# SRainGit/CAE-LO

Hardware: AMD Instinct MI355X
Metric: KITTI frames/sec end-to-end (keypts+desc+match+RANSAC) (higher is better)
Workload: dtype f32

## Files before the change

### cae-lo_amd/csrc/caelo_internal.h

```cpp
#pragma once
#include <hip/hip_runtime.h>
#include <stdint.h>
#include <stdio.h>
#include <string.h>

#include "../../include/caelo.h"

#define CAELO_API extern "C" __attribute__((visibility("default")))

void caelo_set_error(const char *fmt, ...);

#define CAELO_HIP(expr)                                                                     \
    do {                                                                                    \
        hipError_t _e = (expr);                                                             \
        if (_e != hipSuccess) {                                                             \
            caelo_set_error("%s:%d: %s failed: %s", __FILE__, __LINE__, #expr, hipGetErrorString(_e)); \
            return CAELO_ERR_HIP;                                                           \
        }                                                                                   \
    } while (0)

#define CAELO_LAUNCH_CHECK()                                                                \
    do {                                                                                    \
        hipError_t _e = hipGetLastError();                                                  \
        if (_e != hipSuccess) {                                                             \
// ... 188 lines not shown
}
#endif
int certify_record(const caelo_ransac_cert &c, const double *rnd, caelo_pose_result *res, uint8_t *mask, int64_t mask_len, int32_t *evals);

struct caelo_clear_item {
    void *ptr;
    size_t bytes;
    uint32_t pattern;
};
#define CAELO_CLEAR_MAX 12
struct caelo_clear_list {
    caelo_clear_item item[CAELO_CLEAR_MAX];
    int n;
};
int caelo_clear_many(const caelo_clear_list &list, hipStream_t s);
int caelo_clear_many_set(const caelo_clear_list *lists, int n_frames, hipStream_t s);

int ring_project_launch(const float *pc, int64_t n, float *ring, int32_t *counter, int32_t *winner, int32_t *status,
                        hipStream_t s);
int ring_respond_launch(caelo_ctx *c, const float *in, int in_w, int in_c, float *resp, hipStream_t s);
int ring_keypoints_launch(const float *ring, int ring_w, int ring_c, int dist_c, const int32_t *counter, int cnt_w,
                          const float *resp, unsigned long long *cand, int32_t *cand_count,
                          int64_t *key_pixels, float *key_pts, int kp_ld, float *valid, int valid_ld, int32_t *n_key,
                          int32_t *status, hipStream_t s);
int ring_project_set(const caelo_frame_set &fs, hipStream_t s);
int ring_respond_set(caelo_ctx *c, const caelo_frame_set &fs, int in_w, int in_c, hipStream_t s, int row0, int rows);
int ring_keypoints_set(const caelo_frame_set &fs, int ring_w, int ring_c, int cnt_w, hipStream_t s);
void vox_clear_items(caelo_voxmap *m, int level, caelo_clear_list &list);
int vox_clear_for_fast_build(caelo_voxmap *m, caelo_clear_list &list, hipStream_t s);
int vox_clear_for_fast_build_set(caelo_voxmap *const *maps, int n, caelo_clear_list *lists, hipStream_t s);
int vox_build_fast_set(caelo_voxmap *const *maps, const caelo_frame_set &fs, hipStream_t s);
int vox_build_set(caelo_voxmap *const *maps, const caelo_frame_set &fs, bool track_order, hipStream_t s);
int vox_patches_set(const caelo_frame_set &fs, int64_t k_max, bool check_counts, hipStream_t s);
int dedup_set(const caelo_frame_set &fs, bool enabled, hipStream_t s);
int vox_build_launch(caelo_voxmap *m, const float *pc, int64_t n, int stride, bool track_order, int32_t *status,
                     hipStream_t s);
int vox_build_fast_launch(caelo_voxmap *m, const float *pc, int64_t n, int stride, int32_t *status, hipStream_t s);
int vox_patches_launch(const caelo_voxmap *m, const float *pts, int pts_ld, int64_t k_max, const int32_t *n_key,
                       uint64_t *bits, uint8_t *flags, int32_t *status, bool check_counts, hipStream_t s,
                       void *dedup_scratch = nullptr);
#define CAELO_FRAME_PATCHES (CAELO_MAX_KEYPTS * 3)
struct caelo_dedup_tables {
    int32_t count;
    int32_t pad[63];
    int32_t list[CAELO_FRAME_PATCHES];
    int32_t slot_of[CAELO_FRAME_PATCHES];
};
#define CAELO_FRAME_BITS_BYTES ((size_t)CAELO_FRAME_PATCHES * 64 * 8)
#define CAELO_FRAME_BUF_BYTES (CAELO_FRAME_BITS_BYTES + sizeof(caelo_dedup_tables))
__host__ __device__ inline caelo_dedup_tables *caelo_frame_tables(const uint64_t *frame_bits) {
    return (caelo_dedup_tables *)((char *)frame_bits + CAELO_FRAME_BITS_BYTES);
}
#define DD_SLOTS_FRAME 8192
#define DD_SLOTS_SET 65536
#define DD_EMPTY 0xFFFFFFFFFFFFFFFFull
struct DedupScratch {
    unsigned long long table[DD_SLOTS_SET];
    int32_t pslot[CAELO_FRAME_PATCHES];
    int32_t rep[CAELO_FRAME_PATCHES];
};
__host__ __device__ inline uint32_t dedup_slot_mask(int n_frames) { return (n_frames > 1 ? DD_SLOTS_SET : DD_SLOTS_FRAME) - 1; }
int64_t dedup_scratch_bytes();
void dedup_clear_item(void *scratch, int n_frames, caelo_clear_list &list);
unsigned long long dedup_hash_mask();
bool dedup_enabled(int mode);
int dedup_launch(uint64_t *frame_bits, void *scratch, bool enabled, hipStream_t s);

#define CAELO_ENC_MAX_FRAMES CAELO_FB_MAX
struct caelo_enc_out {
    float *base[CAELO_ENC_MAX_FRAMES];
    int64_t per_frame;
};
#define CAELO_ENC_WS_HEADER 4096
#define CAELO_ENC_WS_MFMA 3072
struct caelo_enc_in {
    const unsigned long long *bits;
    int64_t frame_stride;
    int32_t per_frame, n_frames, dedup;
    int32_t yield;
};
__device__ inline const caelo_dedup_tables *enc_tables(const caelo_enc_in &in, int f) {
    return (const caelo_dedup_tables *)(in.bits + (size_t)f * in.frame_stride + (size_t)in.per_frame * 64);
}
int encode_batch_impl(caelo_ctx *c, const uint64_t *bits, int64_t n_patches, int group, const caelo_enc_out &outs,
                      int out_stride, void *ws, hipStream_t s, hipEvent_t *ev, const caelo_enc_in *in = nullptr);
int64_t enc_dense_pad(int64_t n);
int enc_upload_dense1(const float *wd1, const float *bd1, int K, void **wx_dev, float **bd_dev);
int64_t enc_dense32_part_bytes(int64_t np);
int enc_dense32_head_launch(caelo_ctx *c, const float *f3, int64_t n_patches, int64_t np, float *part, int group, float *out,
                            int out_stride, hipStream_t s);
int encode_impl(caelo_ctx *c, const uint64_t *bits, int64_t n_patches, int group, float *out, int out_stride, void *ws,
                hipStream_t s, hipEvent_t *ev);

struct caelo_extract_args {
    caelo_ctx *ctx;
    caelo_voxmap *map;
    const float *pc;
    int64_t n;
    int dist_channels, mode;
    float *key_pts;
    int kp_ld;
    float *features;
    int feat_ld;
    float *valid;
    int valid_ld;
    int64_t *key_pixels;
    int32_t *n_key;
    uint8_t *flags;
    int32_t *status;
    void *ws;
    uint64_t *bits;
};
int extract_check(const caelo_extract_args &a);
int extract_front_launch(const caelo_extract_args &a, hipStream_t s);
int extract_front_set(const caelo_extract_args *args, int n, hipStream_t s, hipStream_t s_vox = nullptr, hipEvent_t ev_fork = nullptr,
                      hipEvent_t ev_join = nullptr);
int extract_encode_launch(const caelo_extract_args &a, hipStream_t s);
int exact_patches_prepare(caelo_voxmap *const *maps, int n_frames);
void exact_patches_clear_item(caelo_voxmap *m, caelo_clear_list &list);
int exact_patches_redo(caelo_voxmap *const *maps, const caelo_frame_set &fs, const caelo_extract_args *args, int n, hipStream_t s);

int correct_prepare(caelo_voxmap *const *maps, int n);
int correct_set(const caelo_extract_args *args, int n, hipStream_t s);

#define CAELO_KP_HIST_BINS 2048

__device__ inline void caelo_frame_block(int n_frames, unsigned &frame, unsigned &block, unsigned &per_frame) {
    per_frame = gridDim.x / (unsigned)n_frames;
    if ((n_frames & (n_frames - 1)) == 0) {
        frame = blockIdx.x & (unsigned)(n_frames - 1);
        block = blockIdx.x / (unsigned)n_frames;
    } else {
        frame = blockIdx.x / per_frame;
        block = blockIdx.x - frame * per_frame;
    }
}

__device__ inline void caelo_lds_barrier() { __asm__ volatile("s_waitcnt lgkmcnt(0)\n\ts_barrier" ::: "memory"); }

__host__ __device__ inline unsigned long long caelo_pack3(int x, int y, int z) {
    return ((unsigned long long)(unsigned)(x & 0xFFFFF) << 40) | ((unsigned long long)(unsigned)(y & 0xFFFFF) << 20) |
           (unsigned long long)(unsigned)(z & 0xFFFFF);
}

__device__ inline uint32_t caelo_hash64(unsigned long long k) {
    k ^= k >> 33;
    k *= 0xff51afd7ed558ccdULL;
    k ^= k >> 33;
    k *= 0xc4ceb9fe1a85ec53ULL;
    k ^= k >> 33;
    return (uint32_t)k;
}

__device__ inline unsigned long long caelo_dd_mix(unsigned long long k) {
    k ^= k >> 33;
    k *= 0xff51afd7ed558ccdULL;
    k ^= k >> 33;
    k *= 0xc4ceb9fe1a85ec53ULL;
    k ^= k >> 33;
    return k;
}
__device__ inline void caelo_dedup_insert(unsigned long long word, int lane, int p, int gp, DedupScratch *S, DedupScratch *T, uint32_t slot_mask,
                                          unsigned long long hash_mask) {
    unsigned long long h = caelo_dd_mix(word + 0x9E3779B97F4A7C15ull * (unsigned)(lane + 1));
#pragma unroll
    for (int o = 32; o > 0; o >>= 1) h += __shfl_xor(h, o);
    if (lane != 0) return;
    h = caelo_dd_mix(h) & hash_mask & 0xFFFFFFFFFEull;
// ... 65 lines not shown
```

### cae-lo_amd/csrc/encoder.hip

```cpp
#include <math.h>

#include "caelo_internal.h"
#include <vector>
#include <stdlib.h>
#include <string.h>

typedef float f32x4 __attribute__((ext_vector_type(4)));

#define MFMA16(a, b, c) __builtin_amdgcn_mfma_f32_16x16x4f32((a), (b), (c), 0, 0, 0)

__device__ inline float enc_tanh(float x) {
    const float e = __builtin_amdgcn_exp2f(x * 2.8853900817779268f);
    return 1.0f - 2.0f * __builtin_amdgcn_rcpf(e + 1.0f);
}

#define DENSE_N 200
#define DENSE_NP 208
#define DENSE_K 2048
#define C3X_NPAIR 14
#define C3X_TICKET_INT 512
static void conv3_split_weights(const float *w3, uint4 *out);
static void stage1x_split_weights(const float *w1, const float *w2, uint4 *w1f, uint4 *w2x);
int enc_upload_dense1(const float *wd1, const float *bd1, int K, void **wx_dev, float **bd_dev);
#define HEAD_WQ_FLOATS (13 * 2 * 64 * 4)
// ... 940 lines not shown
    const float *src = part + (size_t)row * DENSE_NP + 4 * g;
    float4 v[HM_JW][SPLIT];
#pragma unroll
    for (int c = 0; c < HM_JW; ++c)
#pragma unroll
        for (int sp = 0; sp < SPLIT; ++sp)
            if (wave + 4 * c < D1_NT) v[c][sp] = *(const float4 *)(src + (size_t)sp * n_rows_pad * DENSE_NP + 16 * (wave + 4 * c));
    f32x4 acc0 = {0.f, 0.f, 0.f, 0.f}, acc1 = {0.f, 0.f, 0.f, 0.f};
#pragma unroll
    for (int c = 0; c < HM_JW; ++c) {
        if (wave + 4 * c < D1_NT) {
            float4 sum = b1[c];
#pragma unroll
            for (int sp = 0; sp < SPLIT; ++sp) { sum.x += v[c][sp].x; sum.y += v[c][sp].y; sum.z += v[c][sp].z; sum.w += v[c][sp].w; }
            const float hv[4] = {enc_tanh(sum.x), enc_tanh(sum.y), enc_tanh(sum.z), enc_tanh(sum.w)};
            const float w0[4] = {wq[c][0].x, wq[c][0].y, wq[c][0].z, wq[c][0].w}, w1[4] = {wq[c][1].x, wq[c][1].y, wq[c][1].z, wq[c][1].w};
#pragma unroll
            for (int i = 0; i < 4; ++i) {
                acc0 = __builtin_amdgcn_mfma_f32_16x16x4f32(hv[i], w0[i], acc0, 0, 0, 0);
                acc1 = __builtin_amdgcn_mfma_f32_16x16x4f32(hv[i], w1[i], acc1, 0, 0, 0);
            }
        }
    }
    if (wave > 0) {
        s_c[wave - 1][0][lane] = acc0;
        s_c[wave - 1][1][lane] = acc1;
    }
    __syncthreads();
    if (wave > 0) return;
#pragma unroll
    for (int w = 0; w < 3; ++w) {
        acc0 += s_c[w][0][lane];
        acc1 += s_c[w][1][lane];
    }
    const float bo0 = bd2[m], bo1 = m < 4 ? bd2[16 + m] : 0.0f;
#pragma unroll
    for (int i = 0; i < 4; ++i) {
        const unsigned pp = tile * 16u + 4u * (unsigned)g + (unsigned)i;
        if (pp < n_all) {
            const unsigned f = pp / per_out, q = pp - f * per_out, kp = q / (unsigned)group;
            float *dst = outs.base[f] + (size_t)kp * out_stride + (size_t)(q - kp * (unsigned)group) * 20;
            const float d0 = enc_tanh(bo0 + acc0[i]);
            dst[m] = d0;
            if (!(fabsf(d0) <= 1.0f)) atomicAdd(faults, 1);
            if (m < 4) {
                const float d1 = enc_tanh(bo1 + acc1[i]);
                dst[16 + m] = d1;
                if (!(fabsf(d1) <= 1.0f)) atomicAdd(faults, 1);
            }
        }
    }
}

static inline int64_t pad64(int64_t n) { return (n + D1_BM - 1) / D1_BM * D1_BM; }


CAELO_API int64_t caelo_encode_ws_bytes(int64_t n_patches) {
    const int64_t np = pad64(n_patches);
    return CAELO_ENC_WS_HEADER + (np * 1024 + np * 2048 + (int64_t)D1_SPLIT * np * DENSE_NP) * (int64_t)sizeof(float);
}

CAELO_API int caelo_encode_ws_layout(int64_t n_patches, int64_t out[6]) {
    CAELO_REQUIRE(out && n_patches > 0, "caelo_encode_ws_layout: bad argument");
    const int64_t np = pad64(n_patches);
    out[0] = CAELO_ENC_WS_HEADER;
    out[1] = out[0] + np * 1024 * (int64_t)sizeof(float);
    out[2] = out[1] + np * 2048 * (int64_t)sizeof(float);
    out[3] = np;
    out[4] = D1_SPLIT_OF(DENSE_K);
    out[5] = D1_SPLIT;
    return CAELO_OK;
}

int encode_impl(caelo_ctx *c, const uint64_t *bits, int64_t n_patches, int group, float *out, int out_stride,
                       void *ws, hipStream_t s, hipEvent_t *ev ) {
    CAELO_REQUIRE(out, "null argument");
    caelo_enc_out outs;
    outs.base[0] = out;
    outs.per_frame = n_patches > 0 ? n_patches : 1;
    return encode_batch_impl(c, bits, n_patches, group, outs, out_stride, ws, s, ev);
}

int encode_batch_impl(caelo_ctx *c, const uint64_t *bits, int64_t n_patches, int group, const caelo_enc_out &outs,
                      int out_stride, void *ws, hipStream_t s, hipEvent_t *ev , const caelo_enc_in *in) {
    CAELO_REQUIRE(c && bits && ws, "null argument");
    const caelo_enc_in ein = in ? *in : caelo_enc_in{(const unsigned long long *)bits, 0, (int32_t)(n_patches < 0x7FFFFFFF ? n_patches : 0), 1, 0, 0};
    CAELO_REQUIRE(!ein.dedup || (ein.n_frames >= 1 && ein.n_frames <= CAELO_ENC_MAX_FRAMES && ein.per_frame % (3 * D1_BM) == 0 &&
                                 (int64_t)ein.n_frames * ein.per_frame == n_patches),
                  "bad de-duplicated launch");
    CAELO_REQUIRE(outs.per_frame > 0 && (n_patches + outs.per_frame - 1) / outs.per_frame <= CAELO_ENC_MAX_FRAMES, "bad frame table");
    CAELO_REQUIRE(!ein.dedup || ein.per_frame == CAELO_FRAME_PATCHES, "de-duplicated launches hold whole frames of 3072 patches");
    CAELO_REQUIRE(c->has_enc, "encoder weights not set (caelo_set_encoder_weights)");
    CAELO_REQUIRE(n_patches > 0 && n_patches < 0x7FFFFFFF && group >= 1 && out_stride >= group * 20, "bad shape");
    const int64_t np = pad64(n_patches);
    int *work_counter = (int *)ws;
    unsigned long long *mfma_count = (unsigned long long *)((char *)ws + CAELO_ENC_WS_MFMA);
    float *p2 = (float *)((char *)ws + CAELO_ENC_WS_HEADER);
    float *f3 = p2 + np * 1024;
    float *part = f3 + np * 2048;
    if (np > n_patches)
        CAELO_HIP(hipMemsetAsync(f3 + n_patches * 2048, 0, (size_t)(np - n_patches) * 2048 * sizeof(float), s));
    const bool stage1x = !c->enc_reference;
    static int slots1x_slot[CAELO_MAX_DEVICES];
    static bool slots1x_have[CAELO_MAX_DEVICES];
    static std::mutex slots1x_mu;
    const int slots1x = per_device_once(c->device, slots1x_slot, slots1x_have, slots1x_mu, [&] {
        int per_cu = 0, cus = 0;
        if (hipOccupancyMaxActiveBlocksPerMultiprocessor(&per_cu, (const void *)k_enc_stage1x<false>, 256, 0) != hipSuccess ||
            hipDeviceGetAttribute(&cus, hipDeviceAttributeMultiprocessorCount, c->device) != hipSuccess || per_cu * cus <= 0)
            return 512;
        return per_cu * cus;
    });
    int *xcd_counters = (int *)((char *)ws + 1024);
    static int slots1_slot[CAELO_MAX_DEVICES];
    static bool slots1_have[CAELO_MAX_DEVICES];
    static std::mutex slots1_mu;
    const int slots1 = per_device_once(c->device, slots1_slot, slots1_have, slots1_mu, [&] {
        int per_cu = 0, cus = 0;
        if (hipOccupancyMaxActiveBlocksPerMultiprocessor(&per_cu, (const void *)k_enc_stage1, 256, 0) != hipSuccess ||
            hipDeviceGetAttribute(&cus, hipDeviceAttributeMultiprocessorCount, c->device) != hipSuccess || per_cu * cus <= 0)
            return 768;
        return per_cu * cus;
    });
    const int64_t cap1 = (ein.yield & 1) ? (int64_t)slots1 * 4 / 5 : slots1;
    const unsigned g1 = (unsigned)(n_patches < cap1 ? n_patches : cap1);
    if (ev) CAELO_HIP(hipEventRecord(ev[0], s));
    const int order_group = (n_patches % group == 0) ? group : 1;
    if (stage1x) {
        static const int slots_env = getenv("CAELO_S1X_SLOTS") ? atoi(getenv("CAELO_S1X_SLOTS")) : 0;
        const int64_t capx = slots_env > 0 ? slots_env : ((ein.yield & 1) ? (int64_t)slots1x * 2 / 3 : slots1x);
        unsigned gx = (unsigned)(n_patches < capx ? n_patches : capx);
        if (slots_env > 0 && gx < 8u && n_patches >= 8) gx = 8u;
        if (ev) {
            CAELO_HIP(hipMemsetAsync(mfma_count, 0, 1024, s));
            CAELO_HIP(hipEventRecord(ev[0], s));
            k_enc_stage1x<true><<<gx, 256, 0, s>>>(ein, n_patches, order_group, work_counter, (const uint4 *)c->enc_w1f, c->enc_b1,
                                                   (const uint4 *)c->enc_w2x, c->enc_c0, p2, mfma_count);
        } else
            k_enc_stage1x<false><<<gx, 256, 0, s>>>(ein, n_patches, order_group, work_counter, (const uint4 *)c->enc_w1f, c->enc_b1,
                                                    (const uint4 *)c->enc_w2x, c->enc_c0, p2, mfma_count);
        CAELO_LAUNCH_CHECK();
    } else {
        if (ev) CAELO_HIP(hipMemsetAsync(mfma_count, 0, 1024, s));
        k_enc_stage1<<<g1, 256, 0, s>>>(ein, n_patches, order_group, work_counter, c->enc_w1, c->enc_b1, c->enc_w2, c->enc_c0, p2);
        CAELO_LAUNCH_CHECK();
    }
    if (ev) CAELO_HIP(hipEventRecord(ev[1], s));
    const int64_t pairs = (n_patches + 1) / 2;
    const int64_t cap3 = ((ein.yield & 2) ? 256 : ((ein.yield & 4) ? 384 : 512)) * C3X_WGS / 2;
    const unsigned g3 = (unsigned)(pairs < cap3 ? pairs : cap3);
    k_enc_conv3<<<g3, 256, 0, s>>>(p2, n_patches, ein, (const uint4 *)c->enc_w3x, c->enc_b3, f3, work_counter, xcd_counters);
    CAELO_LAUNCH_CHECK();
    if (ev) CAELO_HIP(hipEventRecord(ev[2], s));
    {
        const int rc = dense1_launch<DENSE_K>(c->device, f3, np, c->enc_wd1x, part, ein, s);
        if (rc) return rc;
    }
    if (ev) CAELO_HIP(hipEventRecord(ev[3], s));
    k_enc_head_mfma<D1_SPLIT_OF(DENSE_K)><<<(unsigned)((n_patches + 15) / 16), 256, 0, s>>>(part, n_patches, np, c->enc_bd1, (const float4 *)c->enc_wd2q,
                                                                                       c->enc_bd2, group, outs, out_stride, ein, c->faults);
    CAELO_LAUNCH_CHECK();
    if (ev) CAELO_HIP(hipEventRecord(ev[4], s));
    return CAELO_OK;
}

int64_t enc_dense_pad(int64_t n) { return pad64(n); }
int64_t enc_dense32_part_bytes(int64_t np) { return (int64_t)D1_SPLIT * np * DENSE_NP * (int64_t)sizeof(float); }
int enc_dense32_head_launch(caelo_ctx *c, const float *f3, int64_t n_patches, int64_t np, float *part, int group, float *out,
                            int out_stride, hipStream_t s) {
    const caelo_enc_in plain = {nullptr, 0, (int32_t)n_patches, 1, 0, 0};
    {
        const int rc = dense1_launch<16384>(c->device, f3, np, c->enc32_wd1x, part, plain, s);
        if (rc) return rc;
    }
    caelo_enc_out outs = {};
    outs.base[0] = out;
    outs.per_frame = n_patches;
    k_enc_head_mfma<D1_SPLIT_OF(16384)><<<(unsigned)((n_patches + 15) / 16), 256, 0, s>>>(part, n_patches, np, c->enc32_bd1, (const float4 *)c->enc_wd2q,
                                                                                     c->enc_bd2, group, outs, out_stride, plain, c->faults);
    CAELO_LAUNCH_CHECK();
    return CAELO_OK;
}

CAELO_API int caelo_encode(caelo_ctx *c, const uint64_t *bits, int64_t n_patches, int group, float *out,
                           int out_stride, void *ws, void *stream) {
    return encode_impl(c, bits, n_patches, group, out, out_stride, ws, caelo_stream(stream), nullptr);
}

CAELO_API int caelo_encode_profile(caelo_ctx *c, const uint64_t *bits, int64_t n_patches, int group, float *out,
                                   int out_stride, void *ws, void *stream, float *ms_host) {
    CAELO_REQUIRE(ms_host != nullptr, "null argument");
    hipStream_t s = caelo_stream(stream);
    hipEvent_t ev[5];
    for (int i = 0; i < 5; ++i) CAELO_HIP(hipEventCreate(&ev[i]));
    int rc = encode_impl(c, bits, n_patches, group, out, out_stride, ws, s, ev);
    if (rc == CAELO_OK) {
        CAELO_HIP(hipEventSynchronize(ev[4]));
        for (int i = 0; i < 4; ++i) CAELO_HIP(hipEventElapsedTime(&ms_host[i], ev[i], ev[i + 1]));
        unsigned long long rows = 0, part[128];
        CAELO_HIP(hipMemcpy(part, (char *)ws + CAELO_ENC_WS_MFMA, sizeof(part), hipMemcpyDeviceToHost));
        for (int i = 0; i < 8; ++i) rows += part[16 * i];
        const bool f32_kernel = c->enc_reference;
        ms_host[4] = (float)((double)rows * (f32_kernel ? 6.0 : 1.0) / 1e6);
        ms_host[5] = f32_kernel ? 2.0f * 16 * 16 * 4 : 2.0f * 16 * 16 * 32;
    }
    for (int i = 0; i < 5; ++i) (void)hipEventDestroy(ev[i]);
    return rc;
}

CAELO_API int caelo_set_encoder_reference(caelo_ctx *c, int on) {
    CAELO_REQUIRE(c, "null argument");
    c->enc_reference = on != 0;
    return CAELO_OK;
}
```

### cae-lo_amd/csrc/frame.hip

```cpp
#include "caelo_internal.h"

struct ClearArgs {
    uint4 *ptr[CAELO_CLEAR_MAX];
    unsigned long long end[CAELO_CLEAR_MAX];
    uint32_t pattern[CAELO_CLEAR_MAX];
    int n;
};

struct ClearSet {
    uint4 *ptr[CAELO_FB_MAX][CAELO_CLEAR_MAX];
    unsigned int end[CAELO_FB_MAX][CAELO_CLEAR_MAX];
    uint32_t pattern[CAELO_FB_MAX][CAELO_CLEAR_MAX];
    int n[CAELO_FB_MAX];
};
static_assert(sizeof(ClearSet) <= 3800, "ClearSet must fit the kernel argument segment");

__global__ void __launch_bounds__(256) k_clear_set(const ClearSet a) {
    const int f = blockIdx.y;
    const int n = a.n[f];
    if (n == 0) return;
    const unsigned int total = a.end[f][n - 1];
    for (unsigned int i = blockIdx.x * blockDim.x + threadIdx.x; i < total; i += gridDim.x * blockDim.x) {
        int r = 0;
        while (i >= a.end[f][r]) ++r;
// ... 105 lines not shown
    CAELO_REQUIRE(a.dist_channels == 5 || a.dist_channels == 3, "dist_channels must be 5 (demo mode) or 3 (batch mode)");
    CAELO_REQUIRE(a.kp_ld >= 3 && a.feat_ld >= 60, "bad leading dimension");
    CAELO_REQUIRE(((uintptr_t)a.status & 15u) == 0, "status must be a 16-byte aligned int32[4]");
    CAELO_REQUIRE(!(a.mode & CAELO_EXTRACT_GIVEN_ROWS), "CAELO_EXTRACT_GIVEN_ROWS is a pipeline job mode (rows are given: nothing to extract)");
    if (a.n > a.map->max_points) {
        caelo_set_error("caelo_extract: %lld points exceed the map capacity %lld", (long long)a.n, (long long)a.map->max_points);
        return CAELO_ERR_CAPACITY;
    }
    return CAELO_OK;
}

int extract_front_launch(const caelo_extract_args &a, hipStream_t s) { return extract_front_set(&a, 1, s); }

__global__ void __launch_bounds__(256) k_given_keypts(const caelo_frame_set fs) {
    const caelo_frame_dev &F = fs.f[blockIdx.z];
    const int K = *F.n_key;
    const bool k_ok = K >= 1 && K <= CAELO_MAX_KEYPTS;
    const float lim = (float)CAELO_GIVEN_KEYPTS_RANGE;
    bool bad = !k_ok;
    for (int i = threadIdx.x; i < CAELO_MAX_KEYPTS; i += 256) {
        const bool in = k_ok && i < K;
        if (in) {
            const float *p = F.key_pts + (size_t)F.kp_ld * i;
#pragma unroll
            for (int a = 0; a < 3; ++a) bad = bad || !(fabsf(p[a]) <= lim);
        }
        if (F.valid) F.valid[(size_t)F.valid_ld * i] = in ? 1.0f : 0.0f;
        F.key_pixels[2 * i] = -1;
        F.key_pixels[2 * i + 1] = -1;
    }
    if (__syncthreads_or(bad) && threadIdx.x == 0) {
        atomicOr(F.status, CAELO_ST_BAD_KEYPTS);
        if (!k_ok) *F.n_key = 0;
    }
}

static int given_keypts_set(const caelo_frame_set &fs, hipStream_t s) {
    k_given_keypts<<<dim3(1, 1, fs.n), 256, 0, s>>>(fs);
    CAELO_LAUNCH_CHECK();
    return CAELO_OK;
}

int extract_front_set(const caelo_extract_args *args, int n, hipStream_t s, hipStream_t s_vox, hipEvent_t ev_fork, hipEvent_t ev_join) {
    CAELO_REQUIRE(n >= 1 && n <= CAELO_FB_MAX, "bad frame count");
    const ExtractLayout L = extract_layout();
    const bool exact_pat = (args[0].mode & CAELO_EXTRACT_EXACT_PATCHES) != 0;
    const bool exact_vox = exact_pat || (args[0].mode & CAELO_EXTRACT_EXACT_VOXELS) != 0;
    const bool dd = dedup_enabled(args[0].mode);
    const bool given = (args[0].mode & CAELO_EXTRACT_GIVEN_KEYPTS) != 0;
    const bool correct = (args[0].mode & CAELO_EXTRACT_CORRECT_PC) != 0;
    caelo_frame_set fs = {};
    fs.n = n;
    caelo_clear_list cl[CAELO_FB_MAX];
    caelo_voxmap *maps[CAELO_FB_MAX];
    for (int i = 0; i < n; ++i) {
        CAELO_REQUIRE(args[i].mode == args[0].mode, "the frames of a set share one mode");
        maps[i] = args[i].map;
    }
    int rc = CAELO_OK;
    if (exact_pat && (rc = exact_patches_prepare(maps, n))) return rc;
    if (correct && ((rc = correct_prepare(maps, n)) || (rc = correct_set(args, n, s)))) return rc;
    for (int i = 0; i < n; ++i) {
        const caelo_extract_args &a = args[i];
        char *ws = (char *)a.ws;
        caelo_frame_dev &d = fs.f[i];
        frame_dev_set_map(d, a.map);
        d.pc = correct ? a.map->corr : a.pc; d.n = a.n; d.pc_stride = 4; d.dist_c = a.dist_channels;
        d.ring = (float *)(ws + L.ring); d.counter = nullptr; d.winner = (int32_t *)(ws + L.winner);
        d.resp = (float *)(ws + L.resp); d.cand = (unsigned long long *)(ws + L.cand); d.cand_count = (int32_t *)(ws + L.cand_count);
        d.key_pixels = a.key_pixels; d.key_pts = a.key_pts; d.kp_ld = a.kp_ld; d.valid = a.valid; d.valid_ld = a.valid_ld;
        d.n_key = a.n_key; d.flags = a.flags; d.status = a.status;
        d.bits = (unsigned long long *)(a.bits ? a.bits : (uint64_t *)(ws + L.bits));
        d.dd = dd ? (DedupScratch *)(ws + L.dd) : nullptr;
        cl[i].n = 0;
        cl[i].item[cl[i].n++] = {d.winner, L.cand_count - L.winner, 0xFFFFFFFFu};
        cl[i].item[cl[i].n++] = {d.cand_count, L.ring - L.cand_count, 0u};
        cl[i].item[cl[i].n++] = {a.status, 16, 0u};
        if (exact_vox) vox_clear_items(a.map, exact_pat ? 2 : 1, cl[i]);
        if (exact_pat) exact_patches_clear_item(a.map, cl[i]);
        if (i == 0) dedup_clear_item(ws + L.dd, n, cl[i]);
    }
    if (!exact_vox && (rc = vox_clear_for_fast_build_set(maps, n, cl, s))) return rc;
    if ((rc = caelo_clear_many_set(cl, n, s))) return rc;
    hipStream_t sv = s_vox ? s_vox : s;
    if (s_vox) {
        CAELO_HIP(hipEventRecord(ev_fork, s));
        CAELO_HIP(hipStreamWaitEvent(s_vox, ev_fork, 0));
    }
    if (exact_vox) rc = vox_build_set(maps, fs, exact_pat, sv);
    else rc = vox_build_fast_set(maps, fs, sv);
    if (rc) return rc;
    if (s_vox) CAELO_HIP(hipEventRecord(ev_join, s_vox));
    if (given) {
        if ((rc = given_keypts_set(fs, s))) return rc;
    } else {
        if ((rc = ring_project_set(fs, s))) return rc;
        if ((rc = ring_respond_set(args[0].ctx, fs, CAELO_RING_W, CAELO_RING_C, s, 6, 52))) return rc;
        if ((rc = ring_keypoints_set(fs, CAELO_RING_W, CAELO_RING_C, CAELO_RING_W, s))) return rc;
    }
    if (s_vox) CAELO_HIP(hipStreamWaitEvent(s, ev_join, 0));
    if ((rc = vox_patches_set(fs, CAELO_MAX_KEYPTS, true, s))) return rc;
    if (exact_pat && (rc = exact_patches_redo(maps, fs, args, n, s))) return rc;
    return dedup_set(fs, dd, s);
}

int extract_encode_launch(const caelo_extract_args &a, hipStream_t s) {
    const ExtractLayout L = extract_layout();
    char *ws = (char *)a.ws;
    const uint64_t *bits = a.bits ? a.bits : (const uint64_t *)(ws + L.bits);
    caelo_enc_out outs;
    outs.base[0] = a.features;
    outs.per_frame = CAELO_FRAME_PATCHES;
    const caelo_enc_in in = {(const unsigned long long *)bits, 0, CAELO_FRAME_PATCHES, 1, 1, 0};
    return encode_batch_impl(a.ctx, bits, CAELO_FRAME_PATCHES, 3, outs, a.feat_ld, ws + L.enc, s, nullptr, &in);
}

CAELO_API int caelo_extract(caelo_ctx *c, caelo_voxmap *m, const float *pc, int64_t n, int dist_channels, int mode,
                            float *key_pts, int kp_ld, float *features, int feat_ld, float *valid, int valid_ld,
                            int64_t *key_pixels, int32_t *n_key, uint8_t *flags, int32_t *status, void *wsv,
                            void *stream) {
    const caelo_extract_args a = {c, m, pc, n, dist_channels, mode, key_pts, kp_ld, features, feat_ld, valid, valid_ld,
                                  key_pixels, n_key, flags, status, wsv, nullptr};
    int rc = extract_check(a);
    if (rc) return rc;
    hipStream_t s = caelo_stream(stream);
    if ((rc = extract_front_launch(a, s))) return rc;
    return extract_encode_launch(a, s);
}
```

### cae-lo_amd/csrc/pipeline.hip

```cpp
#include "caelo_internal.h"

#include <condition_variable>
#include <deque>
#include <mutex>
#include <thread>

#include <stdlib.h>

#include <chrono>
#include <vector>

namespace {
inline unsigned local_event_flags() {
    static const bool sys = getenv("CAELO_PIPE_SYSTEM_FENCES") && atoi(getenv("CAELO_PIPE_SYSTEM_FENCES")) != 0;
    return sys ? hipEventDisableTiming : (hipEventDisableTiming | hipEventDisableSystemFence);
}
constexpr int MAX_BUFFERS = 4;
constexpr int64_t FRAME_PATCHES = (int64_t)CAELO_MAX_KEYPTS * 3;

inline int64_t now_ns() {
    return std::chrono::duration_cast<std::chrono::nanoseconds>(std::chrono::steady_clock::now().time_since_epoch()).count();
}
}

struct caelo_pipeline {
    caelo_ctx *ctx = nullptr;
    int batch = 1, n_buffers = 2;
    int64_t max_points = 0;
    hipStream_t sF = nullptr, sE = nullptr, sP = nullptr;
    hipStream_t sV = nullptr;
    hipEvent_t vox_fork = nullptr, vox_join = nullptr;
    caelo_voxmap *maps[CAELO_FB_MAX] = {nullptr};
    void *ws_extract[CAELO_FB_MAX] = {nullptr};
    uint64_t *bits[MAX_BUFFERS] = {nullptr};
    void *enc_ws = nullptr;
    void *ws_match[CAELO_FB_MAX] = {nullptr}, *ws_ransac[CAELO_FB_MAX] = {nullptr};
    hipEvent_t front_done[MAX_BUFFERS] = {nullptr}, enc_done[MAX_BUFFERS] = {nullptr};
    hipEvent_t begun = nullptr, joined[3] = {nullptr};
    static constexpr int EXT_RING = 16;
    hipEvent_t ext_enc[EXT_RING] = {nullptr};
    unsigned n_ext_enc = 0;
    std::vector<hipEvent_t> up_arrived;
    std::vector<hipEvent_t> pair_read;
    std::vector<caelo_frame_job> pending;
    uint64_t n_batches = 0, submitted = 0;
    int since_begin = 0;
    int pace = 1;
    std::vector<int> plan;
    bool have_last = false;
    bool failed = false;
    caelo_frame_job last = {};
    int64_t stat_jobs = 0, stat_issue_ns = 0, stat_batches = 0;
    static constexpr int CERT_RING = 6;
    struct CertItem {
        const caelo_ransac_cert *dev;
        caelo_pose_result *res;
        uint8_t *mask;
        const double *rand_host, *rand_dev;
        int32_t *info;
    };
    struct CertTask {
        CertItem item[CAELO_FB_MAX];
        int n = 0, remaining = 0;
        uint64_t batch_no = 0;
        caelo_ransac_cert *host = nullptr;
        caelo_ransac_cert *host_dev = nullptr;
        hipEvent_t pair_done = nullptr, copied = nullptr;
        int state = 0;
    };
    CertTask cert_ring[CERT_RING];
    hipStream_t sC = nullptr;
    uint64_t cert_seq = 0;
    std::deque<int> cert_issued;
    std::deque<std::pair<int, int>> cert_queue;
    std::mutex cert_mu;
    std::condition_variable cert_cv;
    static constexpr int CERT_THREADS = 8, CERT_THREADS_DEFAULT = 3;
    std::thread cert_thread[CERT_THREADS];
    bool cert_stop = false, cert_started = false;
    bool cert_zero_copy = true;
    int cert_failed = 0;
    int64_t stat_cert_pairs = 0, stat_cert_evals = 0, stat_cert_ns = 0, stat_cert_drain_ns = 0;
};

namespace {

void cert_process(caelo_pipeline *p, int slot, int i, std::vector<double> &draws) {
    caelo_pipeline::CertTask &t = p->cert_ring[slot];
    int failed = !p->cert_zero_copy && hipEventSynchronize(t.copied) != hipSuccess;
    const int64_t t0 = now_ns();
    int32_t evals = 0;
    if (!failed) {
        const caelo_pipeline::CertItem &it = t.item[i];
        int st = certify_record(t.host[i], it.rand_host, it.res, it.mask, CAELO_MAX_KEYPTS, &evals);
        if (st == 1) {
            draws.resize((size_t)CAELO_RANSAC_LEVELS * CAELO_RANSAC_MAX_TRIALS * 4);
            if (hipMemcpy(draws.data(), it.rand_dev, draws.size() * sizeof(double), hipMemcpyDeviceToHost) != hipSuccess) st = -1;
            else st = certify_record(t.host[i], draws.data(), it.res, it.mask, CAELO_MAX_KEYPTS, &evals);
        }
        if (st < 0 || st == 3) failed = 1;
        if (it.info) { it.info[0] = evals; it.info[1] = st; }
    }
    bool last;
    {
        std::lock_guard<std::mutex> lk(p->cert_mu);
        if (failed) p->cert_failed = 1;
        p->stat_cert_pairs += 1;
        p->stat_cert_evals += evals;
        p->stat_cert_ns += now_ns() - t0;
        last = --t.remaining == 0;
        if (last) t.state = 0;
    }
    if (last) p->cert_cv.notify_all();
}

void cert_worker(caelo_pipeline *p) {
    (void)hipSetDevice(p->ctx->device);
    std::vector<double> draws;
    for (;;) {
        std::pair<int, int> w;
// ... 84 lines not shown
    {
        std::unique_lock<std::mutex> lk(p->cert_mu);
        p->cert_cv.wait(lk, [&] { return t.state == 0; });
    }
    ++p->cert_seq;
    t.n = 0;
    *out = &t;
    *slot_out = slot;
    return CAELO_OK;
}

int cert_wait_idle(caelo_pipeline *p) {
    if (!p->cert_started) return CAELO_OK;
    static const bool verbose = getenv("CAELO_PIPE_VERBOSE") != nullptr;
    const int64_t tv0 = now_ns();
    const int rc = cert_drain(p, 0);
    const int64_t tv1 = now_ns();
    {
        std::vector<double> draws;
        for (;;) {
            std::pair<int, int> w(-1, -1);
            {
                std::lock_guard<std::mutex> lk(p->cert_mu);
                if (!p->cert_queue.empty()) { w = p->cert_queue.back(); p->cert_queue.pop_back(); }
            }
            if (w.first < 0) break;
            cert_process(p, w.first, w.second, draws);
        }
    }
    const int64_t tv2 = now_ns();
    std::unique_lock<std::mutex> lk(p->cert_mu);
    p->cert_cv.wait(lk, [&] {
        for (const caelo_pipeline::CertTask &t : p->cert_ring)
            if (t.state != 0) return false;
        return true;
    });
    if (verbose) fprintf(stderr, "cert_wait_idle: drain (pair stages + copies queued) %.1f us, own share %.1f us, wait for the others %.1f us\n",
                         (tv1 - tv0) / 1e3, (tv2 - tv1) / 1e3, (now_ns() - tv2) / 1e3);
    if (rc) return rc;
    if (p->cert_failed) {
        p->cert_failed = 0;
        caelo_set_error("caelo_pipeline: a certificate could not be evaluated on the host (dgesdd failed or the copy did)");
        return CAELO_ERR_HIP;
    }
    return CAELO_OK;
}

int issue_batch_impl(caelo_pipeline *p) {
    const int n = (int)p->pending.size();
    if (n == 0) return CAELO_OK;
    CAELO_REQUIRE(n <= p->batch && n <= CAELO_FB_MAX, "internal: more pending frames than the batch size");
    const int64_t t0 = now_ns();
    const uint64_t k = p->n_batches;
    const int nb = (int)(k % (uint64_t)p->n_buffers);
    const std::vector<caelo_frame_job> &jobs = p->pending;
    const bool rows_given = (jobs[0].mode & CAELO_EXTRACT_GIVEN_ROWS) != 0;
    caelo_extract_args xa[CAELO_FB_MAX];
    for (int i = 0; i < n && !rows_given; ++i) {
        const caelo_frame_job &j = jobs[i];
        xa[i] = {p->ctx, p->maps[i], j.pc, j.n, j.dist_channels, j.mode, j.rows + 60, 64, j.rows, 64, j.rows + 63, 64,
                 j.key_pixels, j.n_key, j.flags, j.status, p->ws_extract[i],
                 p->bits[nb] + (size_t)i * (CAELO_FRAME_BUF_BYTES / 8)};
        const int rc = extract_check(xa[i]);
        if (rc) return rc;
    }
    p->n_batches = k + 1;
    int rc = CAELO_OK;
    if (!rows_given) {
        if (k >= (uint64_t)p->n_buffers) CAELO_HIP(hipStreamWaitEvent(p->sF, p->enc_done[nb], 0));
        if ((rc = extract_front_set(xa, n, p->sF, p->sV, p->vox_fork, p->vox_join))) return rc;
    }
    CAELO_HIP(hipEventRecord(p->front_done[nb], p->sF));
    if (!p->cert_issued.empty()) {
        if ((rc = cert_drain(p, p->pace >= 0 ? 1 : 2))) return rc;
    }
    const int64_t t1 = now_ns();
    if (!rows_given) {
        CAELO_HIP(hipStreamWaitEvent(p->sE, p->front_done[nb], 0));
        caelo_enc_out outs;
        outs.per_frame = FRAME_PATCHES;
        for (int i = 0; i < n; ++i) outs.base[i] = jobs[i].rows;
        static const int yield = getenv("CAELO_ENC_YIELD") ? atoi(getenv("CAELO_ENC_YIELD")) : 5;
        const caelo_enc_in in = {(const unsigned long long *)p->bits[nb], (int64_t)(CAELO_FRAME_BUF_BYTES / 8), (int32_t)FRAME_PATCHES, n, 1, yield};
        rc = encode_batch_impl(p->ctx, p->bits[nb], n * FRAME_PATCHES, 3, outs, 64, p->enc_ws, p->sE, nullptr, &in);
        if (rc) return rc;
    }
    CAELO_HIP(hipEventRecord(p->enc_done[nb], p->sE));
    const int64_t t2 = now_ns();
    caelo_pair_set ps = {};
    ps.faults = p->ctx->faults;
    caelo_pipeline::CertTask *ctask = nullptr;
    int cslot = -1;
    for (int i = 0; i < n; ++i) {
        const caelo_frame_job &j = jobs[i];
        if (j.pair == CAELO_PAIR_NONE) continue;
        const float *prev_rows = j.prev_rows;
        const int32_t *prev_n = j.prev_n_key;
        if (j.pair == CAELO_PAIR_CHAIN) {
            const caelo_frame_job &pj = i > 0 ? jobs[i - 1] : p->last;
            prev_rows = pj.rows;
            prev_n = pj.n_key;
        }
        caelo_pair_dev &d = ps.p[ps.n];
        d.f0 = prev_rows; d.n0 = prev_n; d.f1 = j.rows; d.n1 = j.n_key;
        d.pc0 = prev_rows + 60; d.pc1 = j.rows + 60;
        d.pair_idx = j.pair_idx; d.ws_match = p->ws_match[ps.n]; d.ws_ransac = p->ws_ransac[ps.n];
        d.rand = j.rand; d.result = j.result; d.mask = j.inlier_mask; d.cert = j.cert;
        d.cert_only = j.result_host ? 1 : 0;
        ++ps.n;
        if (j.result_host) {
            if (!ctask && (rc = cert_task(p, &ctask, &cslot))) return rc;
            if (p->cert_zero_copy) {
                ps.p[ps.n - 1].cert = ctask->host_dev + ctask->n;
                ctask->host[ctask->n].magic = 0;
            } else {
                CAELO_REQUIRE(j.cert, "result_host needs cert (CAELO_CERT_ZEROCOPY=0)");
            }
            ctask->item[ctask->n++] = {j.cert, j.result_host, j.mask_host, j.rand_host, j.rand, j.info_host};
        }
    }
    if (ps.n > 0) {
        CAELO_HIP(hipStreamWaitEvent(p->sP, p->enc_done[nb], 0));
        if ((rc = match_set(ps, 64, CAELO_MAX_KEYPTS, 64, CAELO_MAX_KEYPTS, 60, p->sP))) return rc;
        if ((rc = ransac_set(ps, 64, 64, CAELO_MAX_KEYPTS, p->sP))) return rc;
        if (ctask) {
            ctask->batch_no = k;
            CAELO_HIP(hipEventRecord(ctask->pair_done, p->sP));
            ctask->state = 1;
            p->cert_issued.push_back(cslot);
        }
    }
    p->last = jobs[n - 1];
    p->have_last = true;
    p->stat_jobs += n;
    p->stat_batches += 1;
    p->since_begin += 1;
    p->pending.clear();
    const int64_t t3 = now_ns();
    p->stat_issue_ns += t3 - t0;
    if (p->pace >= 0 && p->since_begin > p->pace)
        CAELO_HIP(hipEventSynchronize(p->enc_done[(int)((k - (uint64_t)p->pace) % (uint64_t)p->n_buffers)]));

    static const bool verbose = getenv("CAELO_PIPE_VERBOSE") != nullptr;
    if (verbose) fprintf(stderr, "batch %llu n=%d issue us: front %.1f enc %.1f pair %.1f\n", (unsigned long long)k, n, (t1 - t0) / 1e3, (t2 - t1) / 1e3, (t3 - t2) / 1e3);
    return CAELO_OK;
}

int issue_batch(caelo_pipeline *p) {
    if (p->failed) {
        p->pending.clear();
        caelo_set_error("caelo_pipeline: a batch of this run failed; caelo_pipeline_begin starts a new run");
        return CAELO_ERR_ARG;
    }
    const uint64_t counted = p->n_batches;
    const int rc = issue_batch_impl(p);
    if (rc) {
        p->pending.clear();
        if (p->n_batches != counted) p->failed = true;
    }
    return rc;
}

}

CAELO_API void caelo_pipeline_destroy(caelo_pipeline *p) {
    if (!p) return;
    for (hipStream_t s : {p->sF, p->sE, p->sP, p->sV})
        if (s) (void)hipStreamSynchronize(s);
    if (p->cert_started) {
        (void)cert_wait_idle(p);
        {
            std::lock_guard<std::mutex> lk(p->cert_mu);
            p->cert_stop = true;
        }
        p->cert_cv.notify_all();
        for (std::thread &th : p->cert_thread)
            if (th.joinable()) th.join();
        for (caelo_pipeline::CertTask &t : p->cert_ring) {
            if (t.host) (void)hipHostFree(t.host);
            if (t.pair_done) (void)hipEventDestroy(t.pair_done);
            if (t.copied) (void)hipEventDestroy(t.copied);
        }
        if (p->sC) (void)hipStreamDestroy(p->sC);
    }
    for (int i = 0; i < CAELO_FB_MAX; ++i) {
        if (p->maps[i]) caelo_voxmap_destroy(p->maps[i]);
        for (void *w : {p->ws_extract[i], p->ws_match[i], p->ws_ransac[i]})
            if (w) (void)hipFree(w);
    }
    for (int i = 0; i < MAX_BUFFERS; ++i) {
        if (p->bits[i]) (void)hipFree(p->bits[i]);
        if (p->front_done[i]) (void)hipEventDestroy(p->front_done[i]);
        if (p->enc_done[i]) (void)hipEventDestroy(p->enc_done[i]);
    }
    if (p->enc_ws) (void)hipFree(p->enc_ws);
    if (p->begun) (void)hipEventDestroy(p->begun);
    for (hipEvent_t e : p->joined)
        if (e) (void)hipEventDestroy(e);
    for (hipEvent_t e : p->up_arrived) (void)hipEventDestroy(e);
    for (hipEvent_t e : p->pair_read) (void)hipEventDestroy(e);
    for (hipEvent_t e : {p->vox_fork, p->vox_join})
        if (e) (void)hipEventDestroy(e);
    for (hipEvent_t e : p->ext_enc)
        if (e) (void)hipEventDestroy(e);
    if (p->sV) (void)hipStreamDestroy(p->sV);
    if (p->sP && p->sP != p->sF) (void)hipStreamDestroy(p->sP);
    if (p->sE && p->sE != p->sF) (void)hipStreamDestroy(p->sE);
    if (p->sF) (void)hipStreamDestroy(p->sF);
    delete p;
}

CAELO_API int caelo_pipeline_create(caelo_ctx *c, int batch, int n_buffers, int64_t max_points, caelo_pipeline **out) {
    CAELO_REQUIRE(c && out, "null argument");
    CAELO_REQUIRE(batch >= 1 && batch <= CAELO_FB_MAX && batch <= CAELO_ENC_MAX_FRAMES, "batch must be in [1, 8]");
    CAELO_REQUIRE(n_buffers >= 2 && n_buffers <= MAX_BUFFERS, "n_buffers must be in [2, 4]");
    CAELO_REQUIRE(c->has_resp && c->has_enc, "weights not set");
    CAELO_HIP(hipSetDevice(c->device));
    caelo_pipeline *p = new caelo_pipeline();
    p->ctx = c;
    p->batch = batch;
    p->n_buffers = n_buffers;
    {
        const char *e = getenv("CAELO_PIPE_PACE");
        const int v = e ? atoi(e) : 1;
        p->pace = v < -1 ? -1 : (v >= n_buffers ? n_buffers - 1 : v);
    }
    p->max_points = max_points;
    p->pending.reserve(CAELO_FB_MAX);
    int rc = CAELO_OK;
    auto hip_ok = [&](hipError_t e, const char *what) {
        if (e != hipSuccess && rc == CAELO_OK) {
            caelo_set_error("caelo_pipeline_create: %s failed: %s", what, hipGetErrorString(e));
            rc = CAELO_ERR_HIP;
        }
    };
    const int n_streams = getenv("CAELO_PIPE_STREAMS") ? atoi(getenv("CAELO_PIPE_STREAMS")) : 3;
    hip_ok(hipStreamCreateWithFlags(&p->sF, hipStreamNonBlocking), "hipStreamCreate");
    if (n_streams >= 2) {
        int lo = 0, hi = 0;
        const bool want = !(getenv("CAELO_PIPE_ENC_PRIO") && atoi(getenv("CAELO_PIPE_ENC_PRIO")) == 0);
        if (!want || hipDeviceGetStreamPriorityRange(&lo, &hi) != hipSuccess ||
            hipStreamCreateWithPriority(&p->sE, hipStreamNonBlocking, hi) != hipSuccess) {
            (void)hipGetLastError();
            p->sE = nullptr;
            hip_ok(hipStreamCreateWithFlags(&p->sE, hipStreamNonBlocking), "hipStreamCreate");
        }
    }
    else p->sE = p->sF;
    if (n_streams >= 3) hip_ok(hipStreamCreateWithFlags(&p->sP, hipStreamNonBlocking), "hipStreamCreate");
    else p->sP = p->sF;
    {
        const char *q = getenv("GPU_MAX_HW_QUEUES"), *v = getenv("CAELO_PIPE_VOX_STREAM");
        const bool want = v ? atoi(v) != 0 : (q && atoi(q) >= 8);
        if (n_streams >= 3 && want) {
            hip_ok(hipStreamCreateWithFlags(&p->sV, hipStreamNonBlocking), "hipStreamCreate");
            hip_ok(hipEventCreateWithFlags(&p->vox_fork, local_event_flags()), "hipEventCreate");
            hip_ok(hipEventCreateWithFlags(&p->vox_join, local_event_flags()), "hipEventCreate");
        }
    }
    hip_ok(hipEventCreateWithFlags(&p->begun, local_event_flags()), "hipEventCreate");
    for (hipEvent_t &e : p->ext_enc) hip_ok(hipEventCreateWithFlags(&e, hipEventDisableTiming), "hipEventCreate");
    for (hipEvent_t &e : p->joined) hip_ok(hipEventCreateWithFlags(&e, hipEventDisableTiming), "hipEventCreate");
    for (int i = 0; i < n_buffers; ++i) {
        hip_ok(hipEventCreateWithFlags(&p->front_done[i], local_event_flags()), "hipEventCreate");
        hip_ok(hipEventCreateWithFlags(&p->enc_done[i], hipEventDisableTiming), "hipEventCreate");
        hip_ok(hipMalloc((void **)&p->bits[i], (size_t)batch * CAELO_FRAME_BUF_BYTES), "hipMalloc");
    }
    const size_t xws = (size_t)caelo_extract_ws_bytes(), mws = (size_t)caelo_match_ws_bytes(CAELO_MAX_KEYPTS), rws = (size_t)caelo_ransac_ws_bytes();
    for (int i = 0; i < batch; ++i) {
        hip_ok(hipMalloc(&p->ws_extract[i], xws), "hipMalloc");
        hip_ok(hipMalloc(&p->ws_match[i], mws), "hipMalloc");
        hip_ok(hipMalloc(&p->ws_ransac[i], rws), "hipMalloc");
        if (rc == CAELO_OK) hip_ok(hipMemset(p->ws_extract[i], 0, xws), "hipMemset");
        if (rc == CAELO_OK) hip_ok(hipMemset(p->ws_match[i], 0, mws), "hipMemset");
        if (rc == CAELO_OK) hip_ok(hipMemset(p->ws_ransac[i], 0, rws), "hipMemset");
        if (rc == CAELO_OK) rc = caelo_voxmap_create(c, max_points, &p->maps[i]);
    }
    hip_ok(hipMalloc(&p->enc_ws, (size_t)caelo_encode_ws_bytes(batch * FRAME_PATCHES)), "hipMalloc");
    if (rc == CAELO_OK) hip_ok(hipMemset(p->enc_ws, 0, CAELO_ENC_WS_HEADER), "hipMemset");
    if (rc != CAELO_OK) {
        caelo_pipeline_destroy(p);
        return rc;
    }
    *out = p;
    return CAELO_OK;
}

CAELO_API int caelo_pipeline_batch(const caelo_pipeline *p) { return p ? p->batch : 0; }

CAELO_API int caelo_pipeline_stats(caelo_pipeline *p, int64_t *out_host) {
    CAELO_REQUIRE(p && out_host, "null argument");
    out_host[0] = p->stat_jobs;
    out_host[1] = p->stat_issue_ns;
    out_host[2] = p->stat_batches;
    out_host[3] = p->batch;
    out_host[4] = p->n_buffers;
    out_host[5] = 1 + (p->sE != p->sF) + (p->sP != p->sF) + (p->sV != nullptr);
    p->stat_jobs = p->stat_issue_ns = p->stat_batches = 0;
    return CAELO_OK;
}

CAELO_API int caelo_pipeline_streams(const caelo_pipeline *p, void **out_host) {
    CAELO_REQUIRE(p && out_host, "null argument");
    out_host[0] = (void *)p->sF;
    out_host[1] = (void *)p->sE;
    out_host[2] = (void *)p->sP;
    out_host[3] = (void *)p->sV;
    return CAELO_OK;
}

CAELO_API int caelo_pipeline_cert_stats(caelo_pipeline *p, int64_t *out_host) {
    CAELO_REQUIRE(p && out_host, "null argument");
    std::lock_guard<std::mutex> lk(p->cert_mu);
    out_host[0] = p->stat_cert_pairs;
    out_host[1] = p->stat_cert_evals;
    out_host[2] = p->stat_cert_ns;
    out_host[3] = p->stat_cert_drain_ns;
    p->stat_cert_pairs = p->stat_cert_evals = p->stat_cert_ns = p->stat_cert_drain_ns = 0;
    return CAELO_OK;
}

CAELO_API int caelo_pipeline_begin(caelo_pipeline *p, void *stream) {
    CAELO_REQUIRE(p, "null argument");
    p->pending.clear();
    p->since_begin = 0;
    if (p->cert_started) (void)cert_wait_idle(p);
    if (p->failed) {
        for (hipStream_t s : {p->sF, p->sE, p->sP, p->sV})
            if (s) (void)hipStreamSynchronize(s);
        p->failed = false;
        p->have_last = false;
    }
    CAELO_HIP(hipEventRecord(p->begun, caelo_stream(stream)));
    for (hipStream_t s : {p->sF, p->sE, p->sP}) CAELO_HIP(hipStreamWaitEvent(s, p->begun, 0));
    return CAELO_OK;
}

CAELO_API int caelo_pipeline_get_pace(const caelo_pipeline *p) { return p ? p->pace : 0; }

CAELO_API int caelo_upload_many(void *const *dst, const void *const *src, const size_t *bytes, int n, void *stream) {
    CAELO_REQUIRE(n >= 0 && (n == 0 || (dst && src && bytes)), "caelo_upload_many: null argument");
    for (int i = 0; i < n; ++i) {
        CAELO_REQUIRE(dst[i] && src[i], "caelo_upload_many: null buffer");
        if (bytes[i]) CAELO_HIP(hipMemcpyAsync(dst[i], src[i], bytes[i], hipMemcpyHostToDevice, caelo_stream(stream)));
    }
    return CAELO_OK;
}

// ... 203 lines not shown
```

Baseline: 18770.

## Add selectable encoder pace point and defer voxel-stream fork past keypoint kernels

Result: no change. 18610 (-0.8%).

```diff
diff --git a/cae-lo_amd/csrc/caelo_internal.h b/cae-lo_amd/csrc/caelo_internal.h
--- a/cae-lo_amd/csrc/caelo_internal.h
+++ b/cae-lo_amd/csrc/caelo_internal.h
@@ -294,8 +294,10 @@
 __device__ inline const caelo_dedup_tables *enc_tables(const caelo_enc_in &in, int f) {
     return (const caelo_dedup_tables *)(in.bits + (size_t)f * in.frame_stride + (size_t)in.per_frame * 64);
 }
+enum { CAELO_ENC_PACE_HEAD = 0, CAELO_ENC_PACE_DENSE = 1, CAELO_ENC_PACE_CONV3 = 2, CAELO_ENC_PACE_STAGE1 = 3 };
 int encode_batch_impl(caelo_ctx *c, const uint64_t *bits, int64_t n_patches, int group, const caelo_enc_out &outs,
-                      int out_stride, void *ws, hipStream_t s, hipEvent_t *ev, const caelo_enc_in *in = nullptr);
+                      int out_stride, void *ws, hipStream_t s, hipEvent_t *ev, const caelo_enc_in *in = nullptr,
+                      hipEvent_t pace_ev = nullptr, int pace_at = CAELO_ENC_PACE_HEAD);
 int64_t enc_dense_pad(int64_t n);
 int enc_upload_dense1(const float *wd1, const float *bd1, int K, void **wx_dev, float **bd_dev);
 int64_t enc_dense32_part_bytes(int64_t np);
diff --git a/cae-lo_amd/csrc/encoder.hip b/cae-lo_amd/csrc/encoder.hip
--- a/cae-lo_amd/csrc/encoder.hip
+++ b/cae-lo_amd/csrc/encoder.hip
@@ -1046,8 +1046,10 @@
 }
 
 int encode_batch_impl(caelo_ctx *c, const uint64_t *bits, int64_t n_patches, int group, const caelo_enc_out &outs,
-                      int out_stride, void *ws, hipStream_t s, hipEvent_t *ev , const caelo_enc_in *in) {
+                      int out_stride, void *ws, hipStream_t s, hipEvent_t *ev , const caelo_enc_in *in,
+                      hipEvent_t pace_ev, int pace_at) {
     CAELO_REQUIRE(c && bits && ws, "null argument");
+    if (!pace_ev) pace_at = CAELO_ENC_PACE_HEAD;
     const caelo_enc_in ein = in ? *in : caelo_enc_in{(const unsigned long long *)bits, 0, (int32_t)(n_patches < 0x7FFFFFFF ? n_patches : 0), 1, 0, 0};
     CAELO_REQUIRE(!ein.dedup || (ein.n_frames >= 1 && ein.n_frames <= CAELO_ENC_MAX_FRAMES && ein.per_frame % (3 * D1_BM) == 0 &&
                                  (int64_t)ein.n_frames * ein.per_frame == n_patches),
@@ -1110,17 +1112,20 @@
         CAELO_LAUNCH_CHECK();
     }
     if (ev) CAELO_HIP(hipEventRecord(ev[1], s));
+    if (pace_at == CAELO_ENC_PACE_STAGE1) CAELO_HIP(hipEventRecord(pace_ev, s));
     const int64_t pairs = (n_patches + 1) / 2;
     const int64_t cap3 = ((ein.yield & 2) ? 256 : ((ein.yield & 4) ? 384 : 512)) * C3X_WGS / 2;
     const unsigned g3 = (unsigned)(pairs < cap3 ? pairs : cap3);
     k_enc_conv3<<<g3, 256, 0, s>>>(p2, n_patches, ein, (const uint4 *)c->enc_w3x, c->enc_b3, f3, work_counter, xcd_counters);
     CAELO_LAUNCH_CHECK();
     if (ev) CAELO_HIP(hipEventRecord(ev[2], s));
+    if (pace_at == CAELO_ENC_PACE_CONV3) CAELO_HIP(hipEventRecord(pace_ev, s));
     {
         const int rc = dense1_launch<DENSE_K>(c->device, f3, np, c->enc_wd1x, part, ein, s);
         if (rc) return rc;
     }
     if (ev) CAELO_HIP(hipEventRecord(ev[3], s));
+    if (pace_at == CAELO_ENC_PACE_DENSE) CAELO_HIP(hipEventRecord(pace_ev, s));
     k_enc_head_mfma<D1_SPLIT_OF(DENSE_K)><<<(unsigned)((n_patches + 15) / 16), 256, 0, s>>>(part, n_patches, np, c->enc_bd1, (const float4 *)c->enc_wd2q,
                                                                                        c->enc_bd2, group, outs, out_stride, ein, c->faults);
     CAELO_LAUNCH_CHECK();
diff --git a/cae-lo_amd/csrc/frame.hip b/cae-lo_amd/csrc/frame.hip
--- a/cae-lo_amd/csrc/frame.hip
+++ b/cae-lo_amd/csrc/frame.hip
@@ -211,15 +211,11 @@
     }
     if (!exact_vox && (rc = vox_clear_for_fast_build_set(maps, n, cl, s))) return rc;
     if ((rc = caelo_clear_many_set(cl, n, s))) return rc;
-    hipStream_t sv = s_vox ? s_vox : s;
-    if (s_vox) {
-        CAELO_HIP(hipEventRecord(ev_fork, s));
-        CAELO_HIP(hipStreamWaitEvent(s_vox, ev_fork, 0));
-    }
-    if (exact_vox) rc = vox_build_set(maps, fs, exact_pat, sv);
-    else rc = vox_build_fast_set(maps, fs, sv);
-    if (rc) return rc;
-    if (s_vox) CAELO_HIP(hipEventRecord(ev_join, s_vox));
+    auto build_voxels = [&](hipStream_t sv) {
+        return exact_vox ? vox_build_set(maps, fs, exact_pat, sv) : vox_build_fast_set(maps, fs, sv);
+    };
+    if (s_vox) CAELO_HIP(hipEventRecord(ev_fork, s));
+    else if ((rc = build_voxels(s))) return rc;
     if (given) {
         if ((rc = given_keypts_set(fs, s))) return rc;
     } else {
@@ -227,7 +223,12 @@
         if ((rc = ring_respond_set(args[0].ctx, fs, CAELO_RING_W, CAELO_RING_C, s, 6, 52))) return rc;
         if ((rc = ring_keypoints_set(fs, CAELO_RING_W, CAELO_RING_C, CAELO_RING_W, s))) return rc;
     }
-    if (s_vox) CAELO_HIP(hipStreamWaitEvent(s, ev_join, 0));
+    if (s_vox) {
+        CAELO_HIP(hipStreamWaitEvent(s_vox, ev_fork, 0));
+        if ((rc = build_voxels(s_vox))) return rc;
+        CAELO_HIP(hipEventRecord(ev_join, s_vox));
+        CAELO_HIP(hipStreamWaitEvent(s, ev_join, 0));
+    }
     if ((rc = vox_patches_set(fs, CAELO_MAX_KEYPTS, true, s))) return rc;
     if (exact_pat && (rc = exact_patches_redo(maps, fs, args, n, s))) return rc;
     return dedup_set(fs, dd, s);
diff --git a/cae-lo_amd/csrc/pipeline.hip b/cae-lo_amd/csrc/pipeline.hip
--- a/cae-lo_amd/csrc/pipeline.hip
+++ b/cae-lo_amd/csrc/pipeline.hip
@@ -6,6 +6,7 @@
 #include <thread>
 
 #include <stdlib.h>
+#include <string.h>
 
 #include <chrono>
 #include <vector>
@@ -36,6 +37,9 @@
     void *enc_ws = nullptr;
     void *ws_match[CAELO_FB_MAX] = {nullptr}, *ws_ransac[CAELO_FB_MAX] = {nullptr};
     hipEvent_t front_done[MAX_BUFFERS] = {nullptr}, enc_done[MAX_BUFFERS] = {nullptr};
+    hipEvent_t enc_pace[MAX_BUFFERS] = {nullptr};
+    bool enc_paced[MAX_BUFFERS] = {false};
+    int pace_at = CAELO_ENC_PACE_HEAD;
     hipEvent_t begun = nullptr, joined[3] = {nullptr};
     static constexpr int EXT_RING = 16;
     hipEvent_t ext_enc[EXT_RING] = {nullptr};
@@ -286,9 +290,10 @@
         for (int i = 0; i < n; ++i) outs.base[i] = jobs[i].rows;
         static const int yield = getenv("CAELO_ENC_YIELD") ? atoi(getenv("CAELO_ENC_YIELD")) : 5;
         const caelo_enc_in in = {(const unsigned long long *)p->bits[nb], (int64_t)(CAELO_FRAME_BUF_BYTES / 8), (int32_t)FRAME_PATCHES, n, 1, yield};
-        rc = encode_batch_impl(p->ctx, p->bits[nb], n * FRAME_PATCHES, 3, outs, 64, p->enc_ws, p->sE, nullptr, &in);
+        rc = encode_batch_impl(p->ctx, p->bits[nb], n * FRAME_PATCHES, 3, outs, 64, p->enc_ws, p->sE, nullptr, &in, p->enc_pace[nb], p->pace_at);
         if (rc) return rc;
     }
+    p->enc_paced[nb] = !rows_given && p->pace_at != CAELO_ENC_PACE_HEAD;
     CAELO_HIP(hipEventRecord(p->enc_done[nb], p->sE));
     const int64_t t2 = now_ns();
     caelo_pair_set ps = {};
@@ -342,8 +347,10 @@
     p->pending.clear();
     const int64_t t3 = now_ns();
     p->stat_issue_ns += t3 - t0;
-    if (p->pace >= 0 && p->since_begin > p->pace)
-        CAELO_HIP(hipEventSynchronize(p->enc_done[(int)((k - (uint64_t)p->pace) % (uint64_t)p->n_buffers)]));
+    if (p->pace >= 0 && p->since_begin > p->pace) {
+        const int pb = (int)((k - (uint64_t)p->pace) % (uint64_t)p->n_buffers);
+        CAELO_HIP(hipEventSynchronize(p->enc_paced[pb] ? p->enc_pace[pb] : p->enc_done[pb]));
+    }
 
     static const bool verbose = getenv("CAELO_PIPE_VERBOSE") != nullptr;
     if (verbose) fprintf(stderr, "batch %llu n=%d issue us: front %.1f enc %.1f pair %.1f\n", (unsigned long long)k, n, (t1 - t0) / 1e3, (t2 - t1) / 1e3, (t3 - t2) / 1e3);
@@ -396,6 +403,7 @@
         if (p->bits[i]) (void)hipFree(p->bits[i]);
         if (p->front_done[i]) (void)hipEventDestroy(p->front_done[i]);
         if (p->enc_done[i]) (void)hipEventDestroy(p->enc_done[i]);
+        if (p->enc_pace[i]) (void)hipEventDestroy(p->enc_pace[i]);
     }
     if (p->enc_ws) (void)hipFree(p->enc_ws);
     if (p->begun) (void)hipEventDestroy(p->begun);
@@ -414,7 +422,25 @@
     delete p;
 }
 
+static int pace_from_env(int *batches, int *at) {
+    const char *e = getenv("CAELO_PIPE_PACE");
+    const char *point = e ? strchr(e, '@') : nullptr;
+    if (e && e != point) *batches = atoi(e);
+    if (!point) return CAELO_OK;
+    static const struct { const char *name; int at; } points[] = {{"head", CAELO_ENC_PACE_HEAD}, {"dense", CAELO_ENC_PACE_DENSE},
+                                                                  {"conv3", CAELO_ENC_PACE_CONV3}, {"stage1", CAELO_ENC_PACE_STAGE1}};
+    for (const auto &pt : points)
+        if (!strcmp(point + 1, pt.name)) {
+            *at = pt.at;
+            return CAELO_OK;
+        }
+    caelo_set_error("caelo_pipeline_create: CAELO_PIPE_PACE names the pace point '%s'; known: head, dense, conv3, stage1", point + 1);
+    return CAELO_ERR_ARG;
+}
+
 CAELO_API int caelo_pipeline_create(caelo_ctx *c, int batch, int n_buffers, int64_t max_points, caelo_pipeline **out) {
+    int pace_batches = 1, pace_at = CAELO_ENC_PACE_HEAD;
+    if (const int rc = pace_from_env(&pace_batches, &pace_at)) return rc;
     CAELO_REQUIRE(c && out, "null argument");
     CAELO_REQUIRE(batch >= 1 && batch <= CAELO_FB_MAX && batch <= CAELO_ENC_MAX_FRAMES, "batch must be in [1, 8]");
     CAELO_REQUIRE(n_buffers >= 2 && n_buffers <= MAX_BUFFERS, "n_buffers must be in [2, 4]");
@@ -424,11 +450,8 @@
     p->ctx = c;
     p->batch = batch;
     p->n_buffers = n_buffers;
-    {
-        const char *e = getenv("CAELO_PIPE_PACE");
-        const int v = e ? atoi(e) : 1;
-        p->pace = v < -1 ? -1 : (v >= n_buffers ? n_buffers - 1 : v);
-    }
+    p->pace = pace_batches < -1 ? -1 : (pace_batches >= n_buffers ? n_buffers - 1 : pace_batches);
+    p->pace_at = pace_at;
     p->max_points = max_points;
     p->pending.reserve(CAELO_FB_MAX);
     int rc = CAELO_OK;
@@ -468,6 +491,7 @@
     for (int i = 0; i < n_buffers; ++i) {
         hip_ok(hipEventCreateWithFlags(&p->front_done[i], local_event_flags()), "hipEventCreate");
         hip_ok(hipEventCreateWithFlags(&p->enc_done[i], hipEventDisableTiming), "hipEventCreate");
+        hip_ok(hipEventCreateWithFlags(&p->enc_pace[i], local_event_flags()), "hipEventCreate");
         hip_ok(hipMalloc((void **)&p->bits[i], (size_t)batch * CAELO_FRAME_BUF_BYTES), "hipMalloc");
     }
     const size_t xws = (size_t)caelo_extract_ws_bytes(), mws = (size_t)caelo_match_ws_bytes(CAELO_MAX_KEYPTS), rws = (size_t)caelo_ransac_ws_bytes();
```
